# SalzmanA/fem-libraries

Hardware: AMD Instinct MI355X
Metric: Melements/s assembled + achieved HBM GB/s, 3D P2 elasticity at 1/2/4/8 GPUs (higher is better)
Workload: dtype f64

## Files before the change

fem-libraries_amd/csrc/femasm.hip:

```cpp
#include <hip/hip_runtime.h>
#include <hipcub/hipcub.hpp>

#include <algorithm>
#include <cfloat>
#include <cstdarg>
#include <cstdlib>
#include <cstring>
#include <cstdio>
#include <map>
#include <mutex>
#include <string>
#include <tuple>
#include <type_traits>
#include <utility>
#include <vector>

#include "../../include/femasm.h"
#include "elements.h"

using namespace femasm;

static thread_local std::string g_err;

static int fail(int code, const char* fmt, ...) {
// ... 3562 lines not shown
      const int32_t c = indices[k];
      if (c < 0 || c >= M.nnodes || (k > b0 && indices[k - 1] >= c)) e |= 2;
    }
    const int64_t j0 = adj_ptr[r], j1 = adj_ptr[r + 1];
    if (j1 < j0 || j0 < 0 || j1 > nent) e |= 32;
    for (int64_t j = j0; j < j1 && !(e & 32); ++j) {
      const int32_t p = adj_idx[j];
      if (p < 0 || p >= nent || M.cells[p] != r || (j > j0 && adj_idx[j - 1] >= p)) {
        e |= 32;
        break;
      }
      const int64_t c = p / nn;
      for (int b = 0; b < nn; ++b) {
        const int32_t col = M.cells[c * nn + b];
        int64_t lo = b0, hi = b1 - 1, f = -1;
        while (lo <= hi) {
          const int64_t mid = (lo + hi) >> 1;
          const int32_t v = indices[mid];
          if (v == col) { f = mid; break; }
          if (v < col) lo = mid + 1; else hi = mid - 1;
        }
        if (f < 0) e |= 4;
        else hit[f] = 1;
      }
    }
    if (e) atomicOr(err, e);
  }
}
__global__ void k_check_hits(const uint8_t* __restrict__ hit, int64_t n, int* err) {
  int e = 0;
  for (int64_t i = blockIdx.x * (int64_t)blockDim.x + threadIdx.x; i < n; i += (int64_t)gridDim.x * blockDim.x)
    if (!hit[i]) e = 8;
  if (e) atomicOr(err, e);
}

static int check_pattern(const fa_mesh* mesh, const fa_adjacency* adj, const int64_t* indptr,
                         const int32_t* indices, int64_t nblocks, bool exact, void* stream) {
  int rc = check_mesh(mesh);
  if (rc) return rc;
  if (!adj || !adj->ptr || !adj->idx || !indptr || (!indices && nblocks > 0)) return fail(FA_E_ARG, "null argument");
  if (nblocks < 0) return fail(FA_E_ARG, "negative block count");
  hipStream_t s = (hipStream_t)stream;
  const int64_t n = mesh->nnodes;
  int64_t h[4] = {0, 0, 0, 0};
  HIP_TRY(hipMemcpyAsync(&h[0], indptr, sizeof(int64_t), hipMemcpyDeviceToHost, s));
  HIP_TRY(hipMemcpyAsync(&h[1], indptr + n, sizeof(int64_t), hipMemcpyDeviceToHost, s));
  HIP_TRY(hipMemcpyAsync(&h[2], adj->ptr, sizeof(int64_t), hipMemcpyDeviceToHost, s));
  HIP_TRY(hipMemcpyAsync(&h[3], adj->ptr + n, sizeof(int64_t), hipMemcpyDeviceToHost, s));
  MeshView M{mesh->cells, mesh->geom, mesh->x, mesh->ncells, mesh->nnodes, mesh->nn, mesh->nv, mesh->gdim};
  int* derr = nullptr;
  uint8_t* hit = nullptr;
  HIP_TRY(hipMallocAsync((void**)&derr, sizeof(int), s));
  HIP_TRY(hipMemsetAsync(derr, 0, sizeof(int), s));
  if ((rc = scratch_alloc((void**)&hit, (size_t)std::max<int64_t>(nblocks, 1), s))) return rc;
  HIP_TRY(hipMemsetAsync(hit, 0, (size_t)std::max<int64_t>(nblocks, 1), s));
  if (n > 0) {
    k_check_pattern<<<grid_for(n), 256, 0, s>>>(M, adj->ptr, adj->idx, indptr, indices, nblocks, hit, derr);
    LAUNCH_CHECK();
  }
  if (nblocks > 0 && exact) {
    k_check_hits<<<grid_for(nblocks), 256, 0, s>>>(hit, nblocks, derr);
    LAUNCH_CHECK();
  }
  int herr = 0;
  HIP_TRY(hipMemcpyAsync(&herr, derr, sizeof(int), hipMemcpyDeviceToHost, s));
  HIP_TRY(hipFreeAsync(hit, s));
  HIP_TRY(hipFreeAsync(derr, s));
  HIP_TRY(hipStreamSynchronize(s));
  if (h[0] != 0 || h[1] != nblocks)
    return fail(FA_E_PATTERN, "pattern: indptr[0] = %lld, indptr[nnodes] = %lld for %lld blocks", (long long)h[0],
                (long long)h[1], (long long)nblocks);
  if (h[2] != 0 || h[3] != mesh->ncells * mesh->nn)
    return fail(FA_E_PATTERN, "adjacency: ptr[0] = %lld, ptr[nnodes] = %lld for %lld entries", (long long)h[2],
                (long long)h[3], (long long)(mesh->ncells * mesh->nn));
  if (herr)
    return fail(FA_E_PATTERN, "pattern check failed (bits %d:%s%s%s%s%s)", herr, (herr & 1) ? " indptr" : "",
                (herr & 2) ? " columns out of range or unsorted" : "", (herr & 4) ? " a cell's (row, column) pair missing" : "",
                (herr & 8) ? " a column no cell needs" : "", (herr & 32) ? " adjacency" : "");
  return FA_OK;
}

extern "C" int fa_check_pattern(const fa_mesh* mesh, const fa_adjacency* adj, const int64_t* indptr,
                                const int32_t* indices, int64_t nblocks, void* stream) {
  return check_pattern(mesh, adj, indptr, indices, nblocks, true, stream);
}

constexpr int kSlotCols = 1024;
__global__ __launch_bounds__(64) void k_build_slots(MeshView M, const int64_t* __restrict__ adj_ptr,
                                                    const int32_t* __restrict__ adj_idx,
                                                    const int64_t* __restrict__ indptr,
                                                    const int32_t* __restrict__ indices, uint16_t* __restrict__ slots,
                                                    int* err) {
  __shared__ int32_t cols[kSlotCols];
  const int nn = M.nn;
  const int lane = threadIdx.x;
  for (int64_t r = blockIdx.x; r < M.nnodes; r += gridDim.x) {
    const int64_t b0 = indptr[r], b1 = indptr[r + 1];
    const int64_t nb = b1 - b0;
    if (nb > 65535) {
      if (lane == 0) atomicOr(err, 8);
      continue;
    }
    const bool inl = nb <= kSlotCols;
    __syncthreads();
    if (inl)
      for (int t = lane; t < nb; t += 64) cols[t] = indices[b0 + t];
    __syncthreads();
    const int64_t j0 = adj_ptr[r], nc = (adj_ptr[r + 1] - j0) * nn;
    for (int64_t t = lane; t < nc; t += 64) {
      const int64_t j = j0 + t / nn;
      const int b = (int)(t % nn);
      const int32_t col = M.cells[(int64_t)(adj_idx[j] / nn) * nn + b];
      int64_t lo = 0, hi = nb - 1, s = -1;
      while (lo <= hi) {
        const int64_t mid = (lo + hi) >> 1;
        const int32_t v = inl ? cols[mid] : indices[b0 + mid];
        if (v == col) { s = mid; break; }
        if (v < col) lo = mid + 1; else hi = mid - 1;
      }
      if (s < 0) { atomicOr(err, 1); s = 0; }
      slots[j * nn + b] = (uint16_t)s;
    }
  }
}

extern "C" int fa_plan_slots(const fa_mesh* mesh, const fa_adjacency* adj, const fa_bsr* A, uint16_t* slots,
                             fa_plan* plan, void* stream) {
  int rc = check_mesh(mesh);
  if (rc) return rc;
  if (!adj || !A || !slots || !plan) return fail(FA_E_ARG, "null argument");
  hipStream_t s = (hipStream_t)stream;
  MeshView M{mesh->cells, mesh->geom, mesh->x, mesh->ncells, mesh->nnodes, mesh->nn, mesh->nv, mesh->gdim};
  int* derr = nullptr;
  HIP_TRY(hipMallocAsync((void**)&derr, sizeof(int), s));
  HIP_TRY(hipMemsetAsync(derr, 0, sizeof(int), s));
  if (mesh->nnodes > 0) {
    k_build_slots<<<grid_for(mesh->nnodes, 1), 64, 0, s>>>(M, adj->ptr, adj->idx, A->indptr, A->indices, slots, derr);
    LAUNCH_CHECK();
  }
  int herr = 0;
  HIP_TRY(hipMemcpyAsync(&herr, derr, sizeof(int), hipMemcpyDeviceToHost, s));
  HIP_TRY(hipFreeAsync(derr, s));
  HIP_TRY(hipStreamSynchronize(s));
  if (herr & 8) return fail(FA_E_CAPACITY, "a row holds more than 65535 blocks");
  if (herr) return fail(FA_E_PATTERN, "sparsity pattern misses a (row, column) pair of a cell");
  plan->slots = slots;
  plan->slot_order = 0;
  plan->eadj = nullptr;
  return FA_OK;
}

constexpr int kKempeRounds = 4;
constexpr int kKempeLen = 6;
constexpr int kOrderThreads = 64;
template <int NN, int NSPLIT>
__global__ __launch_bounds__(kOrderThreads) void k_order_slots(const int64_t* __restrict__ row_start,
                                                                const int64_t* __restrict__ indptr,
                                                                const int64_t* __restrict__ adj_ptr, int64_t nchunks,
                                                                int groups_per_chunk, uint16_t* __restrict__ slots,
                                                                const uint16_t* __restrict__ src,
                                                                const uint16_t* __restrict__ eperm, int rounds) {
  constexpr int NBG = NN / NSPLIT, Q = 16;
  __shared__ uint8_t s_res[kOrderThreads][Q][NBG], s_pick[kOrderThreads][Q][NBG], s_cnt[kOrderThreads][NBG][16];
  __shared__ int s_mx[kOrderThreads][NBG], s_nmx[kOrderThreads][NBG];
  auto& res = s_res[threadIdx.x];
  auto& pick = s_pick[threadIdx.x];
  auto& cnt = s_cnt[threadIdx.x];
  auto& mx = s_mx[threadIdx.x];
  auto& nmx = s_nmx[threadIdx.x];
  const int64_t total = nchunks * groups_per_chunk;
  for (int64_t gid = blockIdx.x * (int64_t)blockDim.x + threadIdx.x; gid < total;
       gid += (int64_t)gridDim.x * blockDim.x) {
    const int64_t c = gid / groups_per_chunk;
    const int g = (int)(gid % groups_per_chunk);
    const int64_t r0 = row_start[c], r1 = row_start[c + 1];
    const int64_t a0 = adj_ptr[r0];
    const int na = (int)(adj_ptr[r1] - a0);
    const int nitems = na * NSPLIT;
    const int p0 = Q * g;
    if (p0 >= nitems) continue;
    const int64_t b0 = indptr[r0];
    const int st = gather_perm_stride(na);
    const float inv = 1.0f / (float)na;
    const int nl = min(Q, nitems - p0);
    uint16_t off[Q][NBG];
    int64_t ent[Q];
    int base[Q];
    const uint16_t* rd = eperm ? src : slots;
    for (int t = 0; t < NBG; ++t)
      for (int r = 0; r < 16; ++r) cnt[t][r] = 0;
    for (int q = 0; q < nl; ++q) {
      const int p = p0 + q;
      const int part = p % NSPLIT;
      const int j = eperm ? (int)eperm[a0 + p / NSPLIT] : gather_perm(p / NSPLIT, na, st, inv);
      const int64_t e = a0 + j;
      int64_t lo = r0, hi = r1 - 1;
      while (lo < hi) {
        const int64_t mid = (lo + hi + 1) >> 1;
        if (adj_ptr[mid] <= e) lo = mid; else hi = mid - 1;
      }
      const int rowlo = (int)(indptr[lo] - b0);
      base[q] = eperm ? rowlo : 0;
      const int64_t ein = e * NN + part * NBG;
      ent[q] = (eperm ? a0 + p / NSPLIT : e) * NN + part * NBG;
      for (int t = 0; t < NBG; ++t) {
        off[q][t] = rd[ein + t];
        res[q][t] = (uint8_t)((rowlo + off[q][t]) & 15);
        pick[q][t] = (uint8_t)t;
        ++cnt[t][res[q][t]];
      }
    }
    auto recount = [&](int t) {
      int m = 0, n = 0;
      for (int r = 0; r < 16; ++r) {
        const int v = cnt[t][r];
        if (v > m) { m = v; n = 1; } else if (v == m) ++n;
      }
      mx[t] = m;
      nmx[t] = n;
    };
    auto moved_max = [&](int t, int co, int cn) {
      if (cn + 1 > mx[t]) return cn + 1;
      if (co == mx[t] && nmx[t] == 1 && cn + 1 < mx[t]) return mx[t] - 1;
      return mx[t];
    };
    for (int t = 0; t < NBG; ++t) recount(t);
    auto swap_pick = [&](int q, int t1, int t2) {
      const int ra = res[q][pick[q][t1]], rb = res[q][pick[q][t2]];
      --cnt[t1][ra]; ++cnt[t1][rb]; --cnt[t2][rb]; ++cnt[t2][ra];
      const uint8_t x = pick[q][t1];
      pick[q][t1] = pick[q][t2];
      pick[q][t2] = x;
      recount(t1);
      recount(t2);
    };
    auto descend = [&]() {
      for (int pass = 0; pass < 32; ++pass) {
        bool improved = false;
        for (int q = 0; q < nl; ++q)
          for (int t1 = 0; t1 < NBG; ++t1)
            for (int t2 = t1 + 1; t2 < NBG; ++t2) {
              const int ra = res[q][pick[q][t1]], rb = res[q][pick[q][t2]];
              if (ra == rb) continue;
              const int a1 = cnt[t1][ra], b1 = cnt[t1][rb], a2 = cnt[t2][ra], b2 = cnt[t2][rb];
              const int d = moved_max(t1, a1, b1) + moved_max(t2, b2, a2) - mx[t1] - mx[t2];
              const int sq = 2 * (b1 - a1) + 2 + 2 * (a2 - b2) + 2;
              if (d < 0 || (d == 0 && sq < 0)) {
                swap_pick(q, t1, t2);
                improved = true;
              }
            }
        if (!improved) break;
      }
    };
    descend();
    if constexpr (NBG > 1) {
      auto res_at = [&](int q, int t) { return (int)res[q][pick[q][t]]; };
      for (int round = 0; round < rounds; ++round) {
        bool improved = false;
        for (int t1 = 0; t1 < NBG; ++t1) {
          for (int r = 0; r < 16; ++r) {
            if (cnt[t1][r] < 2) continue;
            int q0 = -1;
            for (int q = 0; q < nl; ++q)
              if (res_at(q, t1) == r) { q0 = q; break; }
            bool done = false;
            for (int t2 = 0; t2 < NBG && !done; ++t2) {
              if (t2 == t1) continue;
              const int before = mx[t1] + mx[t2];
              int path[kKempeLen], len = 0;
              int q = q0;
              while (true) {
                swap_pick(q, t1, t2);
                path[len++] = q;
                const int rn = res_at(q, t1);
                if (cnt[t1][rn] < 2 || len == kKempeLen) break;
                int qn = -1;
                for (int qq = 0; qq < nl && qn < 0; ++qq) {
                  if (res_at(qq, t1) != rn) continue;
                  bool used = false;
                  for (int l = 0; l < len; ++l) used |= path[l] == qq;
                  if (!used) qn = qq;
                }
                if (qn < 0) break;
                q = qn;
              }
              if (mx[t1] + mx[t2] < before) {
                done = improved = true;
              } else {
                for (int l = len - 1; l >= 0; --l) swap_pick(path[l], t1, t2);
              }
            }
            if (done) break;
          }
        }
        if (!improved) break;
        descend();
      }
    }
    for (int q = 0; q < nl; ++q) {
      const int part = (p0 + q) % NSPLIT;
      uint16_t v[NBG];
      for (int t = 0; t < NBG; ++t) {
        const int k = pick[q][t];
        v[t] = (uint16_t)(((part * NBG + k) << 10) | (base[q] + off[q][k]));
      }
      volatile uint16_t* so = slots + ent[q];
      for (int t = 0; t < NBG; ++t) so[t] = v[t];
    }
  }
}

constexpr int kPermThreads = 64;
template <int NN, int NSPLIT, int MQ>
__global__ __launch_bounds__(kPermThreads) void k_plan_perm(const int64_t* __restrict__ row_start,
                                                            const int64_t* __restrict__ indptr,
                                                            const int64_t* __restrict__ adj_ptr,
                                                            const int32_t* __restrict__ adj_idx, int64_t nchunks,
                                                            const uint16_t* __restrict__ src,
                                                            uint16_t* __restrict__ eperm, int32_t* __restrict__ eadj) {
  constexpr int EQ = NSPLIT <= 16 ? 16 / NSPLIT : 1;
  constexpr int TH = MQ <= 16 ? kPermThreads : 16;
  __shared__ uint8_t s_h[TH][MQ][16], s_fill[TH][MQ];
  auto& h = s_h[threadIdx.x];
  auto& fill = s_fill[threadIdx.x];
  for (int64_t c = blockIdx.x * (int64_t)blockDim.x + threadIdx.x; c < nchunks;
       c += (int64_t)gridDim.x * blockDim.x) {
    const int64_t r0 = row_start[c], r1 = row_start[c + 1];
    const int64_t a0 = adj_ptr[r0];
    const int na = (int)(adj_ptr[r1] - a0);
    if (na <= 0) continue;
    const int64_t b0 = indptr[r0];
    const int nq = min((na + EQ - 1) / EQ, MQ);
    for (int q = 0; q < nq; ++q) {
      fill[q] = 0;
      for (int r = 0; r < 16; ++r) h[q][r] = 0;
    }
    const int st = gather_perm_stride(na);
    const float inv = 1.0f / (float)na;
    for (int jj = 0; jj < na; ++jj) {
      const int j = gather_perm(jj, na, st, inv);
      const int64_t e = a0 + j;
      int64_t lo = r0, hi = r1 - 1;
      while (lo < hi) {
        const int64_t mid = (lo + hi + 1) >> 1;
        if (adj_ptr[mid] <= e) lo = mid; else hi = mid - 1;
      }
      const int rowlo = (int)(indptr[lo] - b0);
      uint8_t res[NN];
      for (int b = 0; b < NN; ++b) res[b] = (uint8_t)((rowlo + src[e * NN + b]) & 15);
      int best = -1, bc = 1 << 30;
      for (int q = 0; q < nq; ++q) {
        const int cap = q + 1 < nq ? EQ : na - EQ * (nq - 1);
        if (fill[q] >= cap) continue;
        int cost = 0;
        for (int b = 0; b < NN; ++b) cost += h[q][res[b]];
        if (cost < bc) { bc = cost; best = q; }
      }
      const int pos = best * EQ + fill[best];
      ++fill[best];
      for (int b = 0; b < NN; ++b) ++h[best][res[b]];
      eperm[a0 + pos] = (uint16_t)j;
      eadj[a0 + pos] = adj_idx[e];
    }
  }
}

constexpr int FA_P2TET_NSPLIT = 2;
constexpr int FA_Q2HEX_NSPLIT = 9;
constexpr int FA_Q3HEX_NSPLIT = 32;
constexpr int FA_Q2QUAD_NSPLIT = 1;
constexpr int FA_P1TET_NSPLIT = 1;
constexpr int FA_P1TET_NT = 256;
constexpr int FA_P2TET_NT = 256;
constexpr int FA_Q2QUAD_NT = 128;
__host__ __device__ constexpr int lin_threads(int gd, int nn) {
  return gd == 3 && nn == 4 ? FA_P1TET_NT : gd == 3 && nn == 10 ? FA_P2TET_NT : gd == 2 && nn == 9 ? FA_Q2QUAD_NT : 256;
}
struct SimplexShape {
  int ct, p, nq, gd, nn, nv, nsplit, neo;
};
constexpr SimplexShape kSimplexShapes[4] = {
    {FA_TRIANGLE, 1, 1, 2, 3, 3, 1, 1},
    {FA_TRIANGLE, 2, 3, 2, 6, 3, 2, 2},
    {FA_TETRAHEDRON, 1, 1, 3, 4, 4, FA_P1TET_NSPLIT, FA_P1TET_NSPLIT},
    {FA_TETRAHEDRON, 2, 4, 3, 10, 4, FA_P2TET_NSPLIT, FA_NEO_NSPLIT},
};
static int lin_simplex_nsplit(int ct, int p, int nq, bool affine = false) {
  if (affine && ct == FA_HEXAHEDRON && p == 1 && nq == 8) return 2;
  if (affine && ct == FA_HEXAHEDRON && p == 2 && nq == 27) return FA_Q2HEX_NSPLIT;
  if (affine && ct == FA_HEXAHEDRON && p == 3 && nq == 64) return FA_Q3HEX_NSPLIT;
  if (affine && ct == FA_QUADRILATERAL && p == 1 && nq == 4) return 1;
  if (affine && ct == FA_QUADRILATERAL && p == 2 && nq == 9) return FA_Q2QUAD_NSPLIT;
  if (affine && ct == FA_QUADRILATERAL && p == 3 && nq == 16) return 4;
  for (const SimplexShape& e : kSimplexShapes)
    if (ct == e.ct && p == e.p && nq == e.nq) return e.nsplit;
  return 0;
}
static int neo_nsplit(int ct, int p) {
  for (const SimplexShape& e : kSimplexShapes)
    if (ct == e.ct && p == e.p) return e.neo;
  return 1;
}

extern "C" int fa_plan_order(const fa_mesh* mesh, const fa_adjacency* adj, const fa_bsr* A, int32_t* eadj,
                             fa_plan* plan, void* stream) {
  int rc = check_mesh(mesh);
  if (rc) return rc;
  if (!adj || !A || !plan) return fail(FA_E_ARG, "null argument");
  if (!plan->slots) return fail(FA_E_ARG, "fa_plan_order needs the slot map (fa_plan_slots first)");
  plan->slot_order = 0;
  plan->eadj = nullptr;
  DevTables T;
  if ((rc = get_tables(mesh->cell_type, mesh->degree, -1, &T))) return rc;
  const int ns = (plan->cell_flags & FA_PLAN_NEO) && is_simplex(mesh->cell_type)
                     ? neo_nsplit(mesh->cell_type, mesh->degree)
                     : lin_simplex_nsplit(mesh->cell_type, mesh->degree, T.nq, (plan->cell_flags & FA_PLAN_AFFINE) != 0);
  if (ns == 0 || plan->nchunks <= 0) return FA_OK;
  if (plan->max_blocks >= 1024 || gather_maxb(false, mesh->gdim * mesh->gdim) >= 1024) return FA_OK;
  const int groups = (int)((std::min<int64_t>(std::max<int32_t>(plan->max_adj, 1), kGatherMaxAdj) * ns + 15) / 16);
  const int rounds = (plan->cell_flags & FA_PLAN_ORDER_SEARCH) ? kKempeRounds : 0;
  hipStream_t s = (hipStream_t)stream;
  const int64_t total = plan->nchunks * groups;
  uint16_t* sl = const_cast<uint16_t*>(plan->slots);
  const bool tensor = mesh->cell_type == FA_HEXAHEDRON || mesh->cell_type == FA_QUADRILATERAL;
  const bool posn = eadj != nullptr && 16 % ns == 0 && !(tensor && mesh->nn * mesh->gdim > 32);
  uint16_t *src = nullptr, *eperm = nullptr;
  const int64_t nent = mesh->ncells * mesh->nn;
  const bool small_q = (int64_t)std::max<int32_t>(plan->max_adj, 1) * ns <= 256;
  if (posn) {
    HIP_TRY(hipMallocAsync((void**)&src, sizeof(uint16_t) * nent * mesh->nn, s));
    HIP_TRY(hipMallocAsync((void**)&eperm, sizeof(uint16_t) * nent, s));
    HIP_TRY(hipMemcpyAsync(src, sl, sizeof(uint16_t) * nent * mesh->nn, hipMemcpyDeviceToDevice, s));
  }
#define ORD(NN_, NS_)                                                                                         \
  do {                                                                                                        \
    if (posn && small_q)                                                                                      \
      k_plan_perm<NN_, NS_, 16><<<grid_for(plan->nchunks, kPermThreads), kPermThreads, 0, s>>>(               \
          plan->row_start, A->indptr, adj->ptr, adj->idx, plan->nchunks, src, eperm, eadj);                      \
    else if (posn)                                                                                            \
      k_plan_perm<NN_, NS_, kGatherMaxAdj / (NS_ <= 16 ? 16 / NS_ : 1)><<<grid_for(plan->nchunks, 16), 16, 0, s>>>( \
          plan->row_start, A->indptr, adj->ptr, adj->idx, plan->nchunks, src, eperm, eadj);                      \
    k_order_slots<NN_, NS_><<<grid_for(total, kOrderThreads), kOrderThreads, 0, s>>>(plan->row_start, A->indptr, adj->ptr, plan->nchunks, \
                                                            groups, sl, src, eperm, rounds);                   \
  } while (0)
  bool ok = true;
  if (mesh->nn == 3 && ns == 1) ORD(3, 1);
  else if (mesh->nn == 6 && ns == 2) ORD(6, 2);
  else if (mesh->nn == 4 && ns == 2) ORD(4, 2);
  else if (mesh->nn == 10 && ns == 2) ORD(10, 2);
  else if (mesh->nn == 10 && ns == 5) ORD(10, 5);
  else if (mesh->nn == 10 && ns == 1) ORD(10, 1);
  else if (mesh->nn == 8 && ns == 2) ORD(8, 2);
  else if (mesh->nn == 27 && ns == FA_Q2HEX_NSPLIT) ORD(27, FA_Q2HEX_NSPLIT);
  else if (mesh->nn == 64 && ns == FA_Q3HEX_NSPLIT) ORD(64, FA_Q3HEX_NSPLIT);
  else if (mesh->nn == 4 && ns == 1) ORD(4, 1);
  else if (mesh->nn == 9 && ns == 1) ORD(9, 1);
  else if (mesh->nn == 16 && ns == 4) ORD(16, 4);
  else ok = false;
#undef ORD
  if (src) HIP_TRY(hipFreeAsync(src, s));
  if (eperm) HIP_TRY(hipFreeAsync(eperm, s));
  if (!ok) return FA_OK;
  LAUNCH_CHECK();
  HIP_TRY(hipStreamSynchronize(s));
  plan->slot_order = ns;
  plan->eadj = posn ? eadj : nullptr;
  return FA_OK;
}

template <int GD>
__global__ void k_check_affine(MeshView M, int* nonaffine) {
  constexpr int NV = 1 << GD;
  for (int64_t c = blockIdx.x * (int64_t)blockDim.x + threadIdx.x; c < M.ncells; c += (int64_t)gridDim.x * blockDim.x) {
    const int32_t* g = M.geom + c * NV;
    double x[NV][GD];
#pragma unroll
    for (int v = 0; v < NV; ++v)
#pragma unroll
      for (int i = 0; i < GD; ++i) x[v][i] = M.x[(int64_t)g[v] * GD + i];
    double h = 0.0, dev = 0.0;
#pragma unroll
    for (int v = 1; v < NV; ++v)
#pragma unroll
      for (int i = 0; i < GD; ++i) {
        double pred = x[0][i];
#pragma unroll
        for (int k = 0; k < GD; ++k)
          if ((v >> k) & 1) pred += x[1 << k][i] - x[0][i];
        dev = fmax(dev, fabs(x[v][i] - pred));
        h = fmax(h, fabs(x[v][i] - x[0][i]));
      }
    if (dev > 1e-12 * h) atomicOr(nonaffine, 1);
  }
}

constexpr int64_t kChunkSeg = 2048;
__global__ void k_chunk_seg(const int64_t* __restrict__ ip, const int64_t* __restrict__ ap, int64_t rb0, int64_t n,
                            int64_t maxb, int maxadj, int64_t* __restrict__ tmp, int64_t* __restrict__ cnt,
                            int* __restrict__ st) {
  const int64_t nseg = (n - rb0 + kChunkSeg - 1) / kChunkSeg;
  for (int64_t t = blockIdx.x * (int64_t)blockDim.x + threadIdx.x; t < nseg; t += (int64_t)gridDim.x * blockDim.x) {
    const int64_t r0 = rb0 + t * kChunkSeg, r1 = min(n, r0 + kChunkSeg);
    int64_t* out = tmp + t * kChunkSeg;
    int64_t k = 0, start = r0;
    int mb = 0, ma = 0, bad = INT32_MAX;
    int64_t ipr = ip[r0], apr = ap[r0], ips = ipr, aps = apr;
    out[k++] = r0;
    for (int64_t r = r0; r < r1; ++r) {
      const int64_t ipn = ip[r + 1], apn = ap[r + 1];
      if ((ipn - ipr > maxb || apn - apr > kGatherMaxAdj) && bad == INT32_MAX) bad = (int)(r - rb0);
      if (r > start && (ipn - ips > maxb || apn - aps > maxadj || r + 1 - start > kGatherMaxRows)) {
        out[k++] = r;
        mb = max(mb, (int)(ipr - ips));
        ma = max(ma, (int)(apr - aps));
        start = r;
        ips = ipr;
        aps = apr;
      }
      ipr = ipn;
      apr = apn;
    }
    mb = max(mb, (int)(ipr - ips));
    ma = max(ma, (int)(apr - aps));
    cnt[t] = k;
    atomicMax(&st[0], mb);
    atomicMax(&st[1], ma);
    if (bad != INT32_MAX) atomicMin(&st[2], bad);
  }
}
__global__ void k_chunk_compact(const int64_t* __restrict__ tmp, const int64_t* __restrict__ off, int64_t rb0, int64_t n,
                                int64_t* __restrict__ row_start) {
  const int64_t nrows = n - rb0, nseg = (nrows + kChunkSeg - 1) / kChunkSeg;
  for (int64_t i = blockIdx.x * (int64_t)blockDim.x + threadIdx.x; i < nrows; i += (int64_t)gridDim.x * blockDim.x) {
    const int64_t t = i / kChunkSeg, k = i % kChunkSeg;
    if (off[t] + k < off[t + 1]) row_start[off[t] + k] = tmp[i];
    if (i == 0) row_start[off[nseg]] = n;
  }
}

static int plan_gather(const fa_mesh* mesh, const fa_adjacency* adj, const fa_bsr* A, int64_t* row_start,
                       fa_plan* plan, void* stream, int64_t maxb, int maxadj) {
  int rc = check_mesh(mesh);
  if (rc) return rc;
  if (!adj || !A || !row_start || !plan) return fail(FA_E_ARG, "null argument");
  hipStream_t s = (hipStream_t)stream;
  int64_t rb0 = A->row_begin, re0 = A->row_end;
  if (re0 <= rb0) { rb0 = 0; re0 = mesh->nnodes; }
  if (rb0 < 0 || re0 > mesh->nnodes) return fail(FA_E_ARG, "row window out of range");
  const int64_t n = re0;
  const int64_t nrows = n - rb0;
  const int64_t nseg = (nrows + kChunkSeg - 1) / kChunkSeg;
  int64_t* tmp = nullptr;
  int64_t* cnt = nullptr;
  int* st = nullptr;
  void* scan_tmp = nullptr;
  size_t scan_bytes = 0;
  if ((rc = scratch_alloc((void**)&tmp, sizeof(int64_t) * (size_t)std::max<int64_t>(nrows, 1), s))) return rc;
  if ((rc = scratch_alloc((void**)&cnt, sizeof(int64_t) * (size_t)(nseg + 1), s))) return rc;
  if ((rc = scratch_alloc((void**)&st, sizeof(int) * 4, s))) return rc;
  static const int st0[4] = {0, 0, INT32_MAX, 0};
  HIP_TRY(hipMemcpyAsync(st, st0, sizeof(st0), hipMemcpyHostToDevice, s));
  HIP_TRY(hipMemsetAsync(cnt, 0, sizeof(int64_t) * (size_t)(nseg + 1), s));
  if (nseg > 0) {
    k_chunk_seg<<<grid_for(nseg, 64), 64, 0, s>>>(A->indptr, adj->ptr, rb0, n, maxb, maxadj, tmp, cnt, st);
    LAUNCH_CHECK();
  }
  HIP_TRY(hipcub::DeviceScan::ExclusiveSum(nullptr, scan_bytes, cnt, cnt, (int)(nseg + 1), s));
  if ((rc = scratch_alloc(&scan_tmp, std::max<size_t>(scan_bytes, 16), s))) return rc;
  HIP_TRY(hipcub::DeviceScan::ExclusiveSum(scan_tmp, scan_bytes, cnt, cnt, (int)(nseg + 1), s));
  if (nrows > 0) {
    k_chunk_compact<<<grid_for(nrows), 256, 0, s>>>(tmp, cnt, rb0, n, row_start);
    LAUNCH_CHECK();
  } else {
    HIP_TRY(hipMemcpyAsync(row_start, &rb0, sizeof(int64_t), hipMemcpyHostToDevice, s));
  }
  int64_t total = 0;
  int sth[3] = {0, 0, 0};
  HIP_TRY(hipMemcpyAsync(&total, cnt + nseg, sizeof(int64_t), hipMemcpyDeviceToHost, s));
  HIP_TRY(hipMemcpyAsync(sth, st, sizeof(int) * 3, hipMemcpyDeviceToHost, s));
  HIP_TRY(hipFreeAsync(scan_tmp, s));
  HIP_TRY(hipFreeAsync(tmp, s));
  HIP_TRY(hipFreeAsync(cnt, s));
  HIP_TRY(hipFreeAsync(st, s));
  HIP_TRY(hipStreamSynchronize(s));
  if (sth[2] != INT32_MAX && sth[2] >= 0) {
    int64_t r = rb0 + sth[2], rp[2][2];
    HIP_TRY(hipMemcpy(rp[0], A->indptr + r, sizeof(int64_t) * 2, hipMemcpyDeviceToHost));
    HIP_TRY(hipMemcpy(rp[1], adj->ptr + r, sizeof(int64_t) * 2, hipMemcpyDeviceToHost));
    return fail(FA_E_CAPACITY, "row %lld has %lld blocks / %lld cells (gather caps %lld / %d): use FA_SCATTER",
                (long long)r, (long long)(rp[0][1] - rp[0][0]), (long long)(rp[1][1] - rp[1][0]), (long long)maxb,
                kGatherMaxAdj);
  }
  const int32_t mb = sth[0], ma = sth[1];
  struct { int64_t k; int64_t size() const { return k; } } rs{total + 1};
  plan->nchunks = (int64_t)rs.size() - 1;
  plan->row_start = row_start;
  plan->cell_flags = 0;
  if ((mesh->cell_type == FA_HEXAHEDRON || mesh->cell_type == FA_QUADRILATERAL) && mesh->ncells > 0) {
    MeshView M{mesh->cells, mesh->geom, mesh->x, mesh->ncells, mesh->nnodes, mesh->nn, mesh->nv, mesh->gdim};
    int* dna = nullptr;
    int na_h = 1;
    HIP_TRY(hipMallocAsync((void**)&dna, sizeof(int), s));
    HIP_TRY(hipMemsetAsync(dna, 0, sizeof(int), s));
    if (mesh->gdim == 3) k_check_affine<3><<<grid_for(mesh->ncells), 256, 0, s>>>(M, dna);
    else k_check_affine<2><<<grid_for(mesh->ncells), 256, 0, s>>>(M, dna);
    LAUNCH_CHECK();
    HIP_TRY(hipMemcpyAsync(&na_h, dna, sizeof(int), hipMemcpyDeviceToHost, s));
    HIP_TRY(hipFreeAsync(dna, s));
    HIP_TRY(hipStreamSynchronize(s));
    if (!na_h) plan->cell_flags |= FA_PLAN_AFFINE;
  }
  plan->max_blocks = mb;
  plan->max_adj = ma;
  plan->slots = nullptr;
  plan->slot_order = 0;
  plan->eadj = nullptr;
  plan->corder = nullptr;
  plan->contrib = nullptr;
  plan->chunk_desc = nullptr;
  return FA_OK;
}

extern "C" int fa_plan_gather(const fa_mesh* mesh, const fa_adjacency* adj, const fa_bsr* A, int64_t* row_start,
                              fa_plan* plan, void* stream) {
  if (!mesh) return fail(FA_E_ARG, "null mesh");
  int maxadj = std::min(FA_GATHER_ENTRY_CAP, kGatherMaxAdj);
  if (mesh->cell_type == FA_TRIANGLE || mesh->cell_type == FA_TETRAHEDRON) {
    DevTables T;
    int rc = get_tables(mesh->cell_type, mesh->degree, -1, &T);
    if (rc) return rc;
    const int ns = lin_simplex_nsplit(mesh->cell_type, mesh->degree, T.nq);
    if (ns > 0) {
      maxadj = std::min(maxadj, lin_threads(mesh->gdim, mesh->nn) / ns);
      return plan_gather(mesh, adj, A, row_start, plan, stream, lin_maxb(mesh->gdim, mesh->nn), maxadj);
    }
  }
  if (mesh->cell_type == FA_QUADRILATERAL || (mesh->cell_type == FA_HEXAHEDRON && mesh->degree == 1)) {
    DevTables T;
    int rc = get_tables(mesh->cell_type, mesh->degree, -1, &T);
    if (rc) return rc;
    const int ns = lin_simplex_nsplit(mesh->cell_type, mesh->degree, T.nq, true);
    if (ns > 0 && T.pk) {
      maxadj = std::min(maxadj, lin_threads(mesh->gdim, mesh->nn) / ns);
      return plan_gather(mesh, adj, A, row_start, plan, stream, lin_maxb(mesh->gdim, mesh->nn), maxadj);
    }
  }
  return plan_gather(mesh, adj, A, row_start, plan, stream, gather_maxb(false, mesh->gdim * mesh->gdim), maxadj);
}

extern "C" int fa_plan_gather_form(const fa_mesh* mesh, int32_t kind, const fa_adjacency* adj, const fa_bsr* A,
                                   int64_t* row_start, fa_plan* plan, void* stream) {
  if (!mesh) return fail(FA_E_ARG, "null mesh");
  if (kind != FA_NEO_HOOKEAN) return fa_plan_gather(mesh, adj, A, row_start, plan, stream);
  const int rc = plan_gather(mesh, adj, A, row_start, plan, stream, gather_maxb(true, mesh->gdim * mesh->gdim),
                             256 / neo_nsplit(mesh->cell_type, mesh->degree));
  if (rc == FA_OK) plan->cell_flags |= FA_PLAN_NEO;
  return rc;
}

extern "C" int fa_plan_gather_contrib(const fa_mesh* mesh, const fa_adjacency* adj, const fa_bsr* A,
                                      int64_t* row_start, fa_plan* plan, void* stream) {
  if (!mesh) return fail(FA_E_ARG, "null mesh");
  return plan_gather(mesh, adj, A, row_start, plan, stream, own_maxb(mesh->gdim * mesh->gdim), FA_OWN_CCAP);
}

template <int NN>
__global__ __launch_bounds__(256) void k_plan_contrib(const int32_t* __restrict__ dofmap, const int64_t* __restrict__ row_start,
                                                      int64_t nchunks, const int64_t* __restrict__ indptr,
                                                      const int32_t* __restrict__ indices, const int64_t* __restrict__ adj_ptr,
                                                      const int32_t* __restrict__ adj_idx, const int64_t* __restrict__ cw,
                                                      int32_t* __restrict__ ccells, uint16_t* __restrict__ words, int maxb,
                                                      int* err) {
  constexpr int CCAP = FA_OWN_CCAP, NC = CCAP * NN;
  __shared__ int32_t s_cols[1024];
  __shared__ int32_t s_cnt[1024], s_start[1024];
  __shared__ int32_t s_rowoff[kGatherMaxRows + 1], s_eoff[kGatherMaxRows + 1];
  __shared__ int32_t s_ent[CCAP], s_first[CCAP];
  __shared__ uint8_t s_erow[CCAP], s_eslot[CCAP];
  __shared__ int32_t s_dofs[NC];
  __shared__ int16_t s_pos[NC], s_rank[NC], s_inv[NC];
  __shared__ int s_nslot;
  const int tid = threadIdx.x;
  for (int64_t c = blockIdx.x; c < nchunks; c += gridDim.x) {
    const int64_t r0 = row_start[c], r1 = row_start[c + 1];
    const int64_t b0 = indptr[r0], b1 = indptr[r1], a0 = adj_ptr[r0], a1 = adj_ptr[r1];
    const int nr = (int)(r1 - r0), nb = (int)(b1 - b0), na = (int)(a1 - a0);
    if (nr > kGatherMaxRows || nb > maxb || nb > 1024 || na > CCAP) {
      if (tid == 0) atomicOr(err, 1);
      continue;
    }
    const int n = na * NN;
    const int K = (int)((cw[c + 1] - cw[c]) >> 8) - 1;
    uint16_t* wp = words + cw[c];
    for (int t = tid; t < nb; t += 256) {
      s_cols[t] = indices[b0 + t];
      s_cnt[t] = 0;
    }
    if (tid <= nr) {
      s_rowoff[tid] = (int)(indptr[r0 + tid] - b0);
      s_eoff[tid] = (int)(adj_ptr[r0 + tid] - a0);
    }
    if (tid < na) s_ent[tid] = adj_idx[a0 + tid];
    __syncthreads();
    if (tid < nr)
      for (int j = s_eoff[tid]; j < s_eoff[tid + 1]; ++j) s_erow[j] = (uint8_t)tid;
    for (int t = tid; t < n; t += 256) s_dofs[t] = dofmap[(int64_t)(s_ent[t / NN] / NN) * NN + t % NN];
    if (tid < na) {
      const int cell = s_ent[tid] / NN;
      int f = tid;
      for (int j = 0; j < tid; ++j)
        if (s_ent[j] / NN == cell) { f = j; break; }
      s_first[tid] = f;
    }
    __syncthreads();
    if (tid < na) {
      const int f = s_first[tid];
      int sl = 0;
      for (int j = 0; j < f; ++j) sl += s_first[j] == j;
      s_eslot[tid] = (uint8_t)sl;
      if (f == tid) ccells[c * CCAP + sl] = s_ent[tid] / NN;
    }
    if (tid == 0) {
      int ns = 0;
      for (int j = 0; j < na; ++j) ns += s_first[j] == j;
      s_nslot = ns;
    }
    for (int t = tid; t < n; t += 256) {
      const int j = t / NN, row = s_erow[j];
      const int32_t col = s_dofs[t];
      int p = lds_find(s_cols, s_rowoff[row], s_rowoff[row + 1], col);
      if (p < 0) {
        atomicOr(err, 2);
        p = 0;
      }
      s_pos[t] = (int16_t)p;
      atomicAdd(&s_cnt[p], 1);
// ... 1667 lines not shown
```

Measured before the change: 1513.

## Parallelize slot ordering across 16 lanes with packed counters and DPP reductions

The slot-ordering kernel is rewritten so that each group of 16 items is handled by 16 cooperating lanes instead of one thread. Per-thread shared-memory tables are replaced by nibble- and 5-bit-packed register words, with DPP row rotates, ballots and shuffles doing the counting and max reductions. The Kempe search now always runs instead of only when a plan flag is set. The change also converts scratch buffers in plan_gather to an RAII Scratch wrapper. The aim is to cut shared-memory traffic and serial per-thread work, at the cost of more complex cross-lane control flow and extra search work in the default path.

```diff
diff --git a/fem-libraries_amd/csrc/femasm.hip b/fem-libraries_amd/csrc/femasm.hip
--- a/fem-libraries_amd/csrc/femasm.hip
+++ b/fem-libraries_amd/csrc/femasm.hip
@@ -3738,7 +3738,27 @@
 
 constexpr int kKempeRounds = 4;
 constexpr int kKempeLen = 6;
-constexpr int kOrderThreads = 64;
+constexpr int kOrderThreads = 256;
+template <class W>
+__device__ __forceinline__ int ord_nib(W x, int t) { return (int)(x >> (4 * t)) & 15; }
+template <class W>
+__device__ __forceinline__ int ord_cnt(W x, int t) { return (int)(x >> (5 * t)) & 31; }
+template <class W>
+__device__ __forceinline__ W ord_set(W x, int t, int v) { return (x & ~((W)31 << (5 * t))) | ((W)v << (5 * t)); }
+template <class W>
+__device__ __forceinline__ W ord_swap_nib(W x, int t1, int t2) {
+  const W d = ((x >> (4 * t1)) ^ (x >> (4 * t2))) & (W)15;
+  return x ^ (d << (4 * t1)) ^ (d << (4 * t2));
+}
+template <int I>
+__device__ __forceinline__ int ord_row_ror(int x) {
+  return __builtin_amdgcn_update_dpp(0, x, 0x120 + I, 0xf, 0xf, false);
+}
+template <int I>
+__device__ __forceinline__ int ord_count_eq(int x, int q) {
+  if constexpr (I == 0) return (int)(x == q);
+  else return (int)(ord_row_ror<I>(x) == q) + ord_count_eq<I - 1>(x, q);
+}
 template <int NN, int NSPLIT>
 __global__ __launch_bounds__(kOrderThreads) void k_order_slots(const int64_t* __restrict__ row_start,
                                                                 const int64_t* __restrict__ indptr,
@@ -3747,16 +3767,15 @@
                                                                 const uint16_t* __restrict__ src,
                                                                 const uint16_t* __restrict__ eperm, int rounds) {
   constexpr int NBG = NN / NSPLIT, Q = 16;
-  __shared__ uint8_t s_res[kOrderThreads][Q][NBG], s_pick[kOrderThreads][Q][NBG], s_cnt[kOrderThreads][NBG][16];
-  __shared__ int s_mx[kOrderThreads][NBG], s_nmx[kOrderThreads][NBG];
-  auto& res = s_res[threadIdx.x];
-  auto& pick = s_pick[threadIdx.x];
-  auto& cnt = s_cnt[threadIdx.x];
-  auto& mx = s_mx[threadIdx.x];
-  auto& nmx = s_nmx[threadIdx.x];
+  static_assert(NBG <= 12, "k_order_slots packs a count per step into 5 bits of a 64-bit word");
+  using W = std::conditional_t<NBG <= 6, uint32_t, uint64_t>;
+  const int q = (int)(threadIdx.x & 15);
+  const int gsh = (int)(threadIdx.x & 48);
+  auto gballot = [&](bool pred) { return (uint32_t)(__ballot(pred) >> gsh) & 0xffffu; };
+  auto from = [&](int v, int l) { return __shfl(v, gsh + l); };
   const int64_t total = nchunks * groups_per_chunk;
-  for (int64_t gid = blockIdx.x * (int64_t)blockDim.x + threadIdx.x; gid < total;
-       gid += (int64_t)gridDim.x * blockDim.x) {
+  for (int64_t gid = blockIdx.x * (int64_t)(kOrderThreads / Q) + threadIdx.x / Q; gid < total;
+       gid += (int64_t)gridDim.x * (kOrderThreads / Q)) {
     const int64_t c = gid / groups_per_chunk;
     const int g = (int)(gid % groups_per_chunk);
     const int64_t r0 = row_start[c], r1 = row_start[c + 1];
@@ -3766,19 +3785,19 @@
     const int p0 = Q * g;
     if (p0 >= nitems) continue;
     const int64_t b0 = indptr[r0];
-    const int st = gather_perm_stride(na);
-    const float inv = 1.0f / (float)na;
     const int nl = min(Q, nitems - p0);
-    uint16_t off[Q][NBG];
-    int64_t ent[Q];
-    int base[Q];
-    const uint16_t* rd = eperm ? src : slots;
-    for (int t = 0; t < NBG; ++t)
-      for (int r = 0; r < 16; ++r) cnt[t][r] = 0;
-    for (int q = 0; q < nl; ++q) {
+    const bool valid = q < nl;
+    uint16_t off[NBG];
+    int64_t ent = 0;
+    int base = 0, part = 0;
+    W cur = 0, pk = 0;
+    for (int t = 0; t < NBG; ++t) off[t] = 0;
+    if (valid) {
+      const uint16_t* rd = eperm ? src : slots;
       const int p = p0 + q;
-      const int part = p % NSPLIT;
-      const int j = eperm ? (int)eperm[a0 + p / NSPLIT] : gather_perm(p / NSPLIT, na, st, inv);
+      part = p % NSPLIT;
+      const int st = gather_perm_stride(na);
+      const int j = eperm ? (int)eperm[a0 + p / NSPLIT] : gather_perm(p / NSPLIT, na, st, 1.0f / (float)na);
       const int64_t e = a0 + j;
       int64_t lo = r0, hi = r1 - 1;
       while (lo < hi) {
@@ -3786,112 +3805,132 @@
         if (adj_ptr[mid] <= e) lo = mid; else hi = mid - 1;
       }
       const int rowlo = (int)(indptr[lo] - b0);
-      base[q] = eperm ? rowlo : 0;
+      base = eperm ? rowlo : 0;
       const int64_t ein = e * NN + part * NBG;
-      ent[q] = (eperm ? a0 + p / NSPLIT : e) * NN + part * NBG;
+      ent = (eperm ? a0 + p / NSPLIT : e) * NN + part * NBG;
+#pragma unroll
       for (int t = 0; t < NBG; ++t) {
-        off[q][t] = rd[ein + t];
-        res[q][t] = (uint8_t)((rowlo + off[q][t]) & 15);
-        pick[q][t] = (uint8_t)t;
-        ++cnt[t][res[q][t]];
-      }
-    }
-    auto recount = [&](int t) {
-      int m = 0, n = 0;
-      for (int r = 0; r < 16; ++r) {
-        const int v = cnt[t][r];
-        if (v > m) { m = v; n = 1; } else if (v == m) ++n;
-      }
-      mx[t] = m;
-      nmx[t] = n;
+        off[t] = rd[ein + t];
+        cur |= (W)((rowlo + off[t]) & 15) << (4 * t);
+        pk |= (W)t << (4 * t);
+      }
+    }
+    W cnt = 0, mxp = 0, nmxp = 0;
+#pragma unroll
+    for (int t = 0; t < NBG; ++t) {
+      const int n = ord_count_eq<15>(valid ? ord_nib(cur, t) : 16, q);
+      int m = n;
+      m = max(m, ord_row_ror<1>(m));
+      m = max(m, ord_row_ror<2>(m));
+      m = max(m, ord_row_ror<4>(m));
+      m = max(m, ord_row_ror<8>(m));
+      cnt |= (W)n << (5 * t);
+      mxp |= (W)m << (5 * t);
+      nmxp |= (W)__popc(gballot(n == m)) << (5 * t);
+    }
+    auto moved_max = [](int m, int n, int co, int cn) {
+      if (cn + 1 > m) return cn + 1;
+      if (co == m && n == 1 && cn + 1 < m) return m - 1;
+      return m;
     };
-    auto moved_max = [&](int t, int co, int cn) {
-      if (cn + 1 > mx[t]) return cn + 1;
-      if (co == mx[t] && nmx[t] == 1 && cn + 1 < mx[t]) return mx[t] - 1;
-      return mx[t];
+    auto swap_pick = [&](int l, int t1, int t2, int ra, int rb, int m1, int m2) {
+      if (q == l) {
+        cur = ord_swap_nib(cur, t1, t2);
+        pk = ord_swap_nib(pk, t1, t2);
+      }
+      if (ra == rb) return;
+      const W one1 = (W)1 << (5 * t1), one2 = (W)1 << (5 * t2);
+      if (q == ra) cnt = cnt - one1 + one2;
+      if (q == rb) cnt = cnt + one1 - one2;
+      mxp = ord_set(ord_set(mxp, t1, m1), t2, m2);
+      const int n1 = __popc(gballot(ord_cnt(cnt, t1) == m1)), n2 = __popc(gballot(ord_cnt(cnt, t2) == m2));
+      nmxp = ord_set(ord_set(nmxp, t1, n1), t2, n2);
     };
-    for (int t = 0; t < NBG; ++t) recount(t);
-    auto swap_pick = [&](int q, int t1, int t2) {
-      const int ra = res[q][pick[q][t1]], rb = res[q][pick[q][t2]];
-      --cnt[t1][ra]; ++cnt[t1][rb]; --cnt[t2][rb]; ++cnt[t2][ra];
-      const uint8_t x = pick[q][t1];
-      pick[q][t1] = pick[q][t2];
-      pick[q][t2] = x;
-      recount(t1);
-      recount(t2);
+    auto descend = [&](uint32_t dirty) {
+      uint32_t changed = 0;
+      for (int pass = 0; pass < 32 && dirty; ++pass) {
+        uint32_t now = 0;
+        for (int t1 = 0; t1 < NBG; ++t1)
+          for (int t2 = t1 + 1; t2 < NBG; ++t2) {
+            if (!(((dirty | now) >> t1 | (dirty | now) >> t2) & 1u)) continue;
+            if (ord_cnt(mxp, t1) == 1 && ord_cnt(mxp, t2) == 1) continue;
+            for (int it = 0; it < Q; ++it) {
+              const int ra = ord_nib(cur, t1), rb = ord_nib(cur, t2);
+              const int w = ord_cnt(cnt, t1) | (ord_cnt(cnt, t2) << 8);
+              const int wa = from(w, ra), wb = from(w, rb);
+              const int a1 = wa & 255, a2 = wa >> 8, b1 = wb & 255, b2 = wb >> 8;
+              const int mx1 = ord_cnt(mxp, t1), mx2 = ord_cnt(mxp, t2);
+              const int m1 = moved_max(mx1, ord_cnt(nmxp, t1), a1, b1);
+              const int m2 = moved_max(mx2, ord_cnt(nmxp, t2), b2, a2);
+              const int d = m1 + m2 - mx1 - mx2;
+              const int sq = 2 * (b1 - a1) + 2 + 2 * (a2 - b2) + 2;
+              const uint32_t want = gballot(valid && ra != rb && (d < 0 || (d == 0 && sq < 0)));
+              if (!want) break;
+              const int l = __ffs(want) - 1;
+              const int x = from(ra | (rb << 4) | (m1 << 8) | (m2 << 16), l);
+              swap_pick(l, t1, t2, x & 15, (x >> 4) & 15, (x >> 8) & 255, x >> 16);
+              now |= 1u << t1 | 1u << t2;
+            }
+          }
+        dirty = now;
+        changed |= now;
+      }
+      return changed;
     };
-    auto descend = [&]() {
-      for (int pass = 0; pass < 32; ++pass) {
-        bool improved = false;
-        for (int q = 0; q < nl; ++q)
-          for (int t1 = 0; t1 < NBG; ++t1)
-            for (int t2 = t1 + 1; t2 < NBG; ++t2) {
-              const int ra = res[q][pick[q][t1]], rb = res[q][pick[q][t2]];
-              if (ra == rb) continue;
-              const int a1 = cnt[t1][ra], b1 = cnt[t1][rb], a2 = cnt[t2][ra], b2 = cnt[t2][rb];
-              const int d = moved_max(t1, a1, b1) + moved_max(t2, b2, a2) - mx[t1] - mx[t2];
-              const int sq = 2 * (b1 - a1) + 2 + 2 * (a2 - b2) + 2;
-              if (d < 0 || (d == 0 && sq < 0)) {
-                swap_pick(q, t1, t2);
-                improved = true;
-              }
+    descend((1u << NBG) - 1u);
+    if constexpr (NBG > 1) {
+      uint32_t kd = (1u << NBG) - 1u;
+      for (int round = 0; round < rounds; ++round) {
+        uint32_t improved = 0;
+        for (int t1 = 0; t1 < NBG; ++t1) {
+          const int mx1 = ord_cnt(mxp, t1);
+          if (mx1 < 2 || ord_cnt(nmxp, t1) != 1) continue;
+          const int r = __ffs(gballot(ord_cnt(cnt, t1) == mx1)) - 1;
+          const int q0 = __ffs(gballot(valid && ord_nib(cur, t1) == r)) - 1;
+          for (int t2 = 0; t2 < NBG; ++t2) {
+            if (t2 == t1 || !(((kd | improved) >> t1 | (kd | improved) >> t2) & 1u)) continue;
+            if (from(ord_cnt(cnt, t2), r) >= ord_cnt(mxp, t2)) continue;
+            const int before = mx1 + ord_cnt(mxp, t2);
+            const W cur0 = cur, pk0 = pk, cnt0 = cnt, mxp0 = mxp, nmxp0 = nmxp;
+            uint32_t used = 0;
+            int l = q0;
+            for (int len = 1;; ++len) {
+              const int x = from(ord_nib(cur, t1) | (ord_nib(cur, t2) << 4), l);
+              const int ra = x & 15, rb = x >> 4;
+              const int w = ord_cnt(cnt, t1) | (ord_cnt(cnt, t2) << 8);
+              const int wa = from(w, ra), wb = from(w, rb);
+              const int m1 = moved_max(ord_cnt(mxp, t1), ord_cnt(nmxp, t1), wa & 255, wb & 255);
+              const int m2 = moved_max(ord_cnt(mxp, t2), ord_cnt(nmxp, t2), wb >> 8, wa >> 8);
+              swap_pick(l, t1, t2, ra, rb, m1, m2);
+              used |= 1u << l;
+              if (len == kKempeLen || from(ord_cnt(cnt, t1), rb) < 2) break;
+              const uint32_t next = gballot(valid && ord_nib(cur, t1) == rb) & ~used;
+              if (!next) break;
+              l = __ffs(next) - 1;
             }
-        if (!improved) break;
-      }
-    };
-    descend();
-    if constexpr (NBG > 1) {
-      auto res_at = [&](int q, int t) { return (int)res[q][pick[q][t]]; };
-      for (int round = 0; round < rounds; ++round) {
-        bool improved = false;
-        for (int t1 = 0; t1 < NBG; ++t1) {
-          for (int r = 0; r < 16; ++r) {
-            if (cnt[t1][r] < 2) continue;
-            int q0 = -1;
-            for (int q = 0; q < nl; ++q)
-              if (res_at(q, t1) == r) { q0 = q; break; }
-            bool done = false;
-            for (int t2 = 0; t2 < NBG && !done; ++t2) {
-              if (t2 == t1) continue;
-              const int before = mx[t1] + mx[t2];
-              int path[kKempeLen], len = 0;
-              int q = q0;
-              while (true) {
-                swap_pick(q, t1, t2);
-                path[len++] = q;
-                const int rn = res_at(q, t1);
-                if (cnt[t1][rn] < 2 || len == kKempeLen) break;
-                int qn = -1;
-                for (int qq = 0; qq < nl && qn < 0; ++qq) {
-                  if (res_at(qq, t1) != rn) continue;
-                  bool used = false;
-                  for (int l = 0; l < len; ++l) used |= path[l] == qq;
-                  if (!used) qn = qq;
-                }
-                if (qn < 0) break;
-                q = qn;
-              }
-              if (mx[t1] + mx[t2] < before) {
-                done = improved = true;
-              } else {
-                for (int l = len - 1; l >= 0; --l) swap_pick(path[l], t1, t2);
-              }
+            if (ord_cnt(mxp, t1) + ord_cnt(mxp, t2) < before) {
+              improved |= 1u << t1 | 1u << t2;
+              break;
             }
-            if (done) break;
+            cur = cur0, pk = pk0, cnt = cnt0, mxp = mxp0, nmxp = nmxp0;
           }
         }
         if (!improved) break;
-        descend();
-      }
-    }
-    for (int q = 0; q < nl; ++q) {
-      const int part = (p0 + q) % NSPLIT;
+        kd = improved | descend(improved);
+      }
+    }
+    if (valid) {
       uint16_t v[NBG];
+#pragma unroll
       for (int t = 0; t < NBG; ++t) {
-        const int k = pick[q][t];
-        v[t] = (uint16_t)(((part * NBG + k) << 10) | (base[q] + off[q][k]));
-      }
-      volatile uint16_t* so = slots + ent[q];
+        const int k = ord_nib(pk, t);
+        int o = 0;
+#pragma unroll
+        for (int kk = 0; kk < NBG; ++kk) o = k == kk ? (int)off[kk] : o;
+        v[t] = (uint16_t)(((part * NBG + k) << 10) | (base + o));
+      }
+      volatile uint16_t* so = slots + ent;
+#pragma unroll
       for (int t = 0; t < NBG; ++t) so[t] = v[t];
     }
   }
@@ -4005,7 +4044,7 @@
   if (ns == 0 || plan->nchunks <= 0) return FA_OK;
   if (plan->max_blocks >= 1024 || gather_maxb(false, mesh->gdim * mesh->gdim) >= 1024) return FA_OK;
   const int groups = (int)((std::min<int64_t>(std::max<int32_t>(plan->max_adj, 1), kGatherMaxAdj) * ns + 15) / 16);
-  const int rounds = (plan->cell_flags & FA_PLAN_ORDER_SEARCH) ? kKempeRounds : 0;
+  const int rounds = kKempeRounds;
   hipStream_t s = (hipStream_t)stream;
   const int64_t total = plan->nchunks * groups;
   uint16_t* sl = const_cast<uint16_t*>(plan->slots);
@@ -4027,7 +4066,7 @@
     else if (posn)                                                                                            \
       k_plan_perm<NN_, NS_, kGatherMaxAdj / (NS_ <= 16 ? 16 / NS_ : 1)><<<grid_for(plan->nchunks, 16), 16, 0, s>>>( \
           plan->row_start, A->indptr, adj->ptr, adj->idx, plan->nchunks, src, eperm, eadj);                      \
-    k_order_slots<NN_, NS_><<<grid_for(total, kOrderThreads), kOrderThreads, 0, s>>>(plan->row_start, A->indptr, adj->ptr, plan->nchunks, \
+    k_order_slots<NN_, NS_><<<grid_for(total * 16, kOrderThreads), kOrderThreads, 0, s>>>(plan->row_start, A->indptr, adj->ptr, plan->nchunks, \
                                                             groups, sl, src, eperm, rounds);                   \
   } while (0)
   bool ok = true;
@@ -4137,14 +4176,14 @@
   const int64_t n = re0;
   const int64_t nrows = n - rb0;
   const int64_t nseg = (nrows + kChunkSeg - 1) / kChunkSeg;
-  int64_t* tmp = nullptr;
-  int64_t* cnt = nullptr;
-  int* st = nullptr;
-  void* scan_tmp = nullptr;
+  Scratch tmp_own, cnt_own, st_own, scan_own;
   size_t scan_bytes = 0;
-  if ((rc = scratch_alloc((void**)&tmp, sizeof(int64_t) * (size_t)std::max<int64_t>(nrows, 1), s))) return rc;
-  if ((rc = scratch_alloc((void**)&cnt, sizeof(int64_t) * (size_t)(nseg + 1), s))) return rc;
-  if ((rc = scratch_alloc((void**)&st, sizeof(int) * 4, s))) return rc;
+  if ((rc = tmp_own.alloc(sizeof(int64_t) * (size_t)std::max<int64_t>(nrows, 1), s))) return rc;
+  if ((rc = cnt_own.alloc(sizeof(int64_t) * (size_t)(nseg + 1), s))) return rc;
+  if ((rc = st_own.alloc(sizeof(int) * 4, s))) return rc;
+  int64_t* tmp = tmp_own.as<int64_t>();
+  int64_t* cnt = cnt_own.as<int64_t>();
+  int* st = st_own.as<int>();
   static const int st0[4] = {0, 0, INT32_MAX, 0};
   HIP_TRY(hipMemcpyAsync(st, st0, sizeof(st0), hipMemcpyHostToDevice, s));
   HIP_TRY(hipMemsetAsync(cnt, 0, sizeof(int64_t) * (size_t)(nseg + 1), s));
@@ -4153,8 +4192,8 @@
     LAUNCH_CHECK();
   }
   HIP_TRY(hipcub::DeviceScan::ExclusiveSum(nullptr, scan_bytes, cnt, cnt, (int)(nseg + 1), s));
-  if ((rc = scratch_alloc(&scan_tmp, std::max<size_t>(scan_bytes, 16), s))) return rc;
-  HIP_TRY(hipcub::DeviceScan::ExclusiveSum(scan_tmp, scan_bytes, cnt, cnt, (int)(nseg + 1), s));
+  if ((rc = scan_own.alloc(std::max<size_t>(scan_bytes, 16), s))) return rc;
+  HIP_TRY(hipcub::DeviceScan::ExclusiveSum(scan_own.as<void>(), scan_bytes, cnt, cnt, (int)(nseg + 1), s));
   if (nrows > 0) {
     k_chunk_compact<<<grid_for(nrows), 256, 0, s>>>(tmp, cnt, rb0, n, row_start);
     LAUNCH_CHECK();
@@ -4165,10 +4204,7 @@
   int sth[3] = {0, 0, 0};
   HIP_TRY(hipMemcpyAsync(&total, cnt + nseg, sizeof(int64_t), hipMemcpyDeviceToHost, s));
   HIP_TRY(hipMemcpyAsync(sth, st, sizeof(int) * 3, hipMemcpyDeviceToHost, s));
-  HIP_TRY(hipFreeAsync(scan_tmp, s));
-  HIP_TRY(hipFreeAsync(tmp, s));
-  HIP_TRY(hipFreeAsync(cnt, s));
-  HIP_TRY(hipFreeAsync(st, s));
+  if ((rc = scan_own.free()) || (rc = tmp_own.free()) || (rc = cnt_own.free()) || (rc = st_own.free())) return rc;
   HIP_TRY(hipStreamSynchronize(s));
   if (sth[2] != INT32_MAX && sth[2] >= 0) {
     int64_t r = rb0 + sth[2], rp[2][2];
```

New measurement: 1528 (median of 6 runs). Within noise of the previous version (+1.0%).
